# semicolonTransistor/rust-ray-tracing

Measured on AMD Instinct MI355X. Metric: Msamples/s (pixels×spp/s), 1920×1080·512spp·500 spheres; 1/2/4/8 GPU, higher is better.
Workload: dtype f32

## Files before the change

rust-ray-tracing_amd/csrc/rt_trace.hpp:

```cpp
#pragma once
#include "rt_sweep.hpp"
#include "rt_camera.hpp"
#include "rt_finish.hpp"

namespace rt {

struct IssueState { uint32_t busy, cur, cur_next, cur_pix, cur_row, cur_col, drained, qhead, qcount, blk_next, blk_end, need; };
struct IssueStateS { uint32_t busy, cur, cur_next, cur_pix, cur_row, cur_col, drained, qhead, qcount, blk_next, blk_end, need, cur_end; };

constexpr uint32_t kMaxBlock = 16;
constexpr uint32_t kBlockShare = 24;
constexpr uint32_t kClaimSpp = 640;
constexpr uint32_t kStreams = 8;
constexpr uint32_t kCtrStride = 64;

__device__ __forceinline__ bool guided_block(uint32_t np, uint32_t T, uint32_t G, uint32_t j, uint32_t& start,
                                             uint32_t& end) {
    uint32_t a = 0;
#pragma unroll
    for (uint32_t sz = kMaxBlock; sz >= 1u; sz >>= 1) {
        const uint32_t r = np - a, keep = sz * T;
        const uint32_t len = sz == 1u ? r : (sz <= G && r > keep ? ((r - keep) / sz) * sz : 0u);
        const uint32_t nb = len / sz;
        if (j < nb) { start = a + j * sz; end = start + sz; return true; }
        j -= nb;
        a += len;
    }
    return false;
}

constexpr uint32_t kQCap = 128;

template <typename T, bool B> constexpr bool kSplitKernel = B;

template <typename T, int W, bool ROOT2, int MODE = kModeV2, bool CAMQ = false, bool MEGA = false>
__global__ __launch_bounds__(256, W) void trace_paths(KParams<T> p) {
    constexpr bool SPLIT = kSplitKernel<T, false>, WIN = kSplitKernel<T, false>, ITEMS = kSplitKernel<T, false>;
    constexpr bool RAYS = kSplitKernel<T, false>;
#include "rt_trace_body.hpp"
}

template <typename T, int W, bool CAMQ, bool MEGA>
__global__ __launch_bounds__(256, W) void trace_paths_split(SParams<T> sp) {
    constexpr bool SPLIT = kSplitKernel<T, true>, WIN = kSplitKernel<T, false>, ITEMS = kSplitKernel<T, false>, ROOT2 = false;
    constexpr bool RAYS = kSplitKernel<T, false>;
    constexpr int MODE = kModeV2;
    const KParams<T>& p = sp.k;
#include "rt_trace_body.hpp"
}

template <typename T, int W, bool CAMQ, bool MEGA>
__global__ __launch_bounds__(256, W) void trace_paths_window(WParams<T> wp) {
    constexpr bool SPLIT = kSplitKernel<T, true>, WIN = kSplitKernel<T, true>, ITEMS = kSplitKernel<T, false>, ROOT2 = false;
    constexpr bool RAYS = kSplitKernel<T, false>;
    constexpr int MODE = kModeV2;
    const KParams<T>& p = wp.s.k;
#include "rt_trace_body.hpp"
}

template <typename T, int W, bool CAMQ, bool MEGA>
__global__ __launch_bounds__(256, W) void trace_paths_items(IParams<T> ip) {
    constexpr bool SPLIT = kSplitKernel<T, true>, WIN = kSplitKernel<T, false>, ITEMS = kSplitKernel<T, true>, ROOT2 = false;
    constexpr bool RAYS = kSplitKernel<T, false>;
    constexpr int MODE = kModeV2;
    const KParams<T>& p = ip.w.s.k;
#include "rt_trace_body.hpp"
}

template <typename T>
__global__ __launch_bounds__(256) void finish_records(SParams<T> sp) {
    __shared__ __attribute__((aligned(16))) uint32_t s_hist[4][64];
    __shared__ __attribute__((aligned(16))) T s_stage[4][3][64];
    __shared__ __attribute__((aligned(16))) uint16_t s_lmap[4][kLMapCap > 0u ? kLMapCap : 2];
    const uint32_t lane = threadIdx.x & 63u;
    const uint32_t wave = __builtin_amdgcn_readfirstlane(threadIdx.x >> 6);
    const auto& q = *cold_split_args<T>();
    const uint32_t gw = blockIdx.x * 4u + wave, nw = gridDim.x * 4u;
    const RScratch<T> sc{q.k.scratch + (size_t)gw * q.k.scratch_stride, q.rec, q.k.P, q.k.sbytes, q.k.swide};
    const uint32_t n_pix = q.n_pix;
    unsigned long long iters = 0;
    for (uint64_t px = gw; px < n_pix; px += nw) {
        iters += finish_pixel<T, kModeV2, true>(sc, (uint32_t)px, (uint32_t)px, s_hist[wave], s_stage[wave],
                                                kLMapCap > 0u ? s_lmap[wave] : nullptr, false);
        __builtin_amdgcn_wave_barrier();
    }
    if (lane == 0 && iters != 0ull) atomicAdd(&q.k.segs[(gw & (kSegShards - 1)) * kSegStride + 2], iters);
}

template <typename T>
__global__ __launch_bounds__(256) void finish_window(WParams<T> wp) {
    __shared__ __attribute__((aligned(16))) uint32_t s_hist[4][64];
    __shared__ __attribute__((aligned(16))) T s_stage[4][3][64];
    __shared__ __attribute__((aligned(16))) uint16_t s_lmap[4][kLMapCap > 0u ? kLMapCap : 2];
    const uint32_t lane = threadIdx.x & 63u;
    const uint32_t wave = __builtin_amdgcn_readfirstlane(threadIdx.x >> 6);
    const auto& q = *cold_split_args<T>();
    const uint32_t gw = blockIdx.x * 4u + wave, nw = gridDim.x * 4u;
    const RScratch<T> sc{q.k.scratch + (size_t)gw * q.k.scratch_stride, q.rec, cold_window_args<T>()->P_cap, q.k.sbytes,
                         q.k.swide};
    const uint32_t n_pix = q.n_pix;
    unsigned long long iters = 0;
    for (uint64_t px = gw; px < n_pix; px += nw) {
        iters += finish_pixel<T, kModeV2, true>(sc, (uint32_t)px, (uint32_t)px, s_hist[wave], s_stage[wave],
                                                kLMapCap > 0u ? s_lmap[wave] : nullptr, false);
        __builtin_amdgcn_wave_barrier();
    }
    if (lane == 0 && iters != 0ull) atomicAdd(&q.k.segs[(gw & (kSegShards - 1)) * kSegStride + 2], iters);
}

template <typename T>
__global__ __launch_bounds__(256) void finish_window_list(LParams<T> lp) {
    __shared__ __attribute__((aligned(16))) uint32_t s_hist[4][64];
    __shared__ __attribute__((aligned(16))) T s_stage[4][3][64];
    __shared__ __attribute__((aligned(16))) uint16_t s_lmap[4][kLMapCap > 0u ? kLMapCap : 2];
    const uint32_t lane = threadIdx.x & 63u;
    const uint32_t wave = __builtin_amdgcn_readfirstlane(threadIdx.x >> 6);
    const auto& q = *cold_split_args<T>();
    const uint32_t gw = blockIdx.x * 4u + wave, nw = gridDim.x * 4u;
    const RScratch<T> sc{q.k.scratch + (size_t)gw * q.k.scratch_stride, q.rec, cold_window_args<T>()->P_cap, q.k.sbytes,
                         q.k.swide};
    const uint32_t n_list = q.n_pix;
    const cptr<uint32_t> list = (cptr<uint32_t>)cold_list_args<T>()->list;
    unsigned long long iters = 0;
    for (uint64_t i = gw; i < n_list; i += nw) {
        const uint32_t px = list[i];
        iters += finish_pixel<T, kModeV2, true>(sc, px, px, s_hist[wave], s_stage[wave],
                                                kLMapCap > 0u ? s_lmap[wave] : nullptr, false);
        __builtin_amdgcn_wave_barrier();
    }
    if (lane == 0 && iters != 0ull) atomicAdd(&q.k.segs[(gw & (kSegShards - 1)) * kSegStride + 2], iters);
}

__global__ __launch_bounds__(256) void progressive_error(const double* full, const double* half,
                                                         const uint32_t* counts, double* out, uint32_t n) {
    const uint32_t i = blockIdx.x * 256u + threadIdx.x;
    if (i >= n) return;
    double e = __builtin_huge_val();
    if (counts[i] >= 2u) {
        e = 0.0;
        for (uint32_t ch = 0; ch < 3u; ++ch) e = fmax(e, fabs(full[3u * i + ch] - half[3u * i + ch]));
    }
    out[i] = e;
}

constexpr uint32_t kRefineBlock = 256;

__device__ inline uint32_t refine_block_scan(uint32_t v, uint32_t* buf, uint32_t* total) {
    const uint32_t t = threadIdx.x;
    buf[t] = v;
    __syncthreads();
    for (uint32_t d = 1; d < kRefineBlock; d <<= 1) {
        const uint32_t a = t >= d ? buf[t - d] : 0u;
        __syncthreads();
        buf[t] += a;
        __syncthreads();
    }
    const uint32_t incl = buf[t];
    *total = buf[kRefineBlock - 1];
    __syncthreads();
    return incl - v;
}

__global__ __launch_bounds__(256) void refine_select(const uint32_t* list, uint32_t n, uint32_t count, double tol,
                                                     uint32_t may_grow, double* cur, const double* fresh,
                                                     uint32_t* counts, uint8_t* flags, uint32_t* blk) {
    __shared__ uint32_t s_buf[kRefineBlock];
    const uint32_t i = blockIdx.x * kRefineBlock + threadIdx.x;
    uint32_t act = 0u;
    if (i < n) {
        const size_t p = list ? list[i] : i;
        double e = __builtin_huge_val();
        if (count >= 2u) {
            e = 0.0;
            for (uint32_t ch = 0; ch < 3u; ++ch) e = fmax(e, fabs(fresh[3u * p + ch] - cur[3u * p + ch]));
        }
        for (uint32_t ch = 0; ch < 3u; ++ch) cur[3u * p + ch] = fresh[3u * p + ch];
        act = (e > tol && may_grow != 0u) ? 1u : 0u;
        counts[p] = count;
        flags[i] = (uint8_t)act;
    }
    uint32_t total = 0u;
    (void)refine_block_scan(act, s_buf, &total);
    if (threadIdx.x == 0u) blk[blockIdx.x] = total;
}

__global__ __launch_bounds__(256) void refine_scan(uint32_t* blk, uint32_t nb, uint32_t* ret) {
    __shared__ uint32_t s_buf[kRefineBlock];
    uint32_t carry = 0u;
    for (uint32_t base = 0; base < nb; base += kRefineBlock) {
        const uint32_t idx = base + threadIdx.x;
        const uint32_t v = idx < nb ? blk[idx] : 0u;
        uint32_t total = 0u;
        const uint32_t ex = refine_block_scan(v, s_buf, &total);
        if (idx < nb) blk[idx] = carry + ex;
        carry += total;
    }
    if (threadIdx.x < 4u) ret[threadIdx.x] = threadIdx.x == 0u ? carry : 0u;
}

__global__ __launch_bounds__(256) void refine_scatter(const uint32_t* list, uint32_t n, const uint8_t* flags,
                                                      const uint32_t* off, uint32_t* next, uint32_t* retired) {
    __shared__ uint32_t s_buf[kRefineBlock];
    const uint32_t first = blockIdx.x * kRefineBlock, i = first + threadIdx.x;
    const uint32_t act = i < n ? (uint32_t)flags[i] : 0u;
    uint32_t total = 0u;
    const uint32_t rank = refine_block_scan(act, s_buf, &total);
    if (i >= n) return;
    const uint32_t p = list ? list[i] : i;
    const uint32_t a0 = off[blockIdx.x];
    if (act) next[a0 + rank] = p;
    else retired[(first - a0) + (threadIdx.x - rank)] = p;
}

__global__ __launch_bounds__(256) void refine_expand(const uint32_t* act, uint32_t n_act, uint32_t* counts,
                                                     uint32_t done, uint32_t target, uint32_t base, uint32_t S,
                                                     uint32_t nsub, MapItem* items) {
    const uint32_t i = blockIdx.x * kRefineBlock + threadIdx.x;
    if (i >= n_act) return;
    const uint32_t p = act[i];
    counts[p] = target;
    for (uint32_t j = 0; j < nsub; ++j) {
        const uint32_t a = base + j * S, b = a + S;
        items[(size_t)i * nsub + j] = MapItem{p, a > done ? a : done, b < target ? b : target, 0u};
    }
}

}
```

rust-ray-tracing_amd/csrc/rt_trace_body.hpp:

```cpp
    constexpr bool SC = MODE == kModeScalar;
    static_assert(!SPLIT || (MODE == kModeV2 && !ROOT2), "the sample-parallel kernels cover the live path only");
    static_assert(!ITEMS || (SPLIT && !WIN), "an item table replaces the window's decode");
    static_assert(!RAYS || (!SPLIT && !CAMQ && MODE == kModeV2), "caller rays: the live path, one item per pixel, no camera batches");
    constexpr bool kF64Park = sizeof(T) == 8 && W >= 5;
    constexpr uint32_t QW = CAMQ ? 4 : 1, QN = CAMQ ? (kF64Park ? 64u : kQCap) : 1;
    __shared__ unsigned long long wcount[4][4];
    __shared__ __attribute__((aligned(16))) uint32_t s_hist[4][64];
    __shared__ __attribute__((aligned(16))) T s_stage[4][3][64];
    using IS = std::conditional_t<SPLIT, IssueStateS, IssueState>;
    __shared__ IS s_is[4];
    __shared__ unsigned long long s_pool;
    __shared__ uint32_t s_dry;
    __shared__ uint32_t q_sid[QW][QN];
    __shared__ uint32_t s_slotpix[4][kSlots];
    __shared__ uint32_t s_item[4][kSlots];
    __shared__ int q_hit[QW][QN];
    __shared__ T q_t[QW][QN], q_d[QW][3][QN];
    __shared__ alignas(16) uint16_t s_clist[QW][CAMQ ? kSlots : 1][kCList];
    constexpr bool kPark = (sizeof(T) == 4 && W >= 6) || kF64Park;
    constexpr bool kParkC = kPark && (MEGA || (sizeof(T) == 4 && W == 6));
    __shared__ T s_park[kPark ? 4 : 1][kParkC ? 9 : 6][64];
    constexpr bool kLMap = MODE == kModeV2 && !MEGA && kLMapCap > 0u && sizeof(T) == 8 && !kF64Park;
    __shared__ __attribute__((aligned(16))) uint16_t s_lmap[kLMap ? 4 : 1][kLMap ? kLMapCap : 2];
    const uint32_t lane = threadIdx.x & 63u;
    const uint32_t wave = __builtin_amdgcn_readfirstlane(threadIdx.x >> 6);
    if (lane == 0) { wcount[wave][0] = 0; wcount[wave][1] = 0; wcount[wave][2] = 0; wcount[wave][3] = 0; }
    if (lane < kNWork) g_work[wave][lane] = 0ull;
#ifdef RT_KSTATS
    if (lane < kNKstat) g_kst[wave][lane] = 0;
#endif
    if constexpr (SPLIT) {
        if (lane == 0) s_is[wave] = IssueStateS{};
    } else {
        if (lane == 0) s_is[wave] = IssueState{0u, 0u, cold_args<T>()->spp, 0u, 0u, 0u, 0u, 0u, 0u, 0u, 0u, 0u};
    }
    {
        const auto& q = *cold_args<T>();
        uint32_t b0 = 0, b1 = 0;
        const bool got = guided_block(q.n_items, max(1u, kTMul * gridDim.x), q.blk_g, blockIdx.x, b0, b1);
        if (threadIdx.x == 0) {
            s_pool = got ? ((unsigned long long)b0 << 32) | b1 : 0ull;
            s_dry = 0u;
        }
    }
    __syncthreads();
    V3<T> o = mk(T(0), T(0), T(0)), d = o, c = o;
    uint32_t ss = 0, k = 0;
    constexpr bool kParkSS = MEGA;
    uint32_t* const ssp = (uint32_t*)&s_stage[wave][0][0] + lane;
    auto ss_get = [&]() -> uint32_t {
        if constexpr (kParkSS) { asm volatile("" ::: "memory"); return *ssp; }
        else return ss;
    };
    auto ss_set = [&](uint32_t v) {
        if constexpr (kParkSS) *ssp = v;
        else ss = v;
    };
    if constexpr (kParkSS) *ssp = 0u;
    constexpr uint32_t kSlotNZ = 0x80000000u;
    uint32_t slot_left = 0;
    auto sid_of = [](uint32_t v) -> uint32_t { return v & 0x1FFFFFFFu; };
    auto slot_of = [](uint32_t v) -> uint32_t { return v >> 29; };
    bool live = false;
    bool scat = false;
    int hit_i = -1;
    T hit_t = T(0);
    auto park = [&](const V3<T>& po, const V3<T>& pd) {
        T* r = &s_park[kPark ? wave : 0][0][lane];
        r[0] = po.x; r[64] = po.y; r[128] = po.z; r[192] = pd.x; r[256] = pd.y; r[320] = pd.z;
    };
    auto unpark = [&](V3<T>& po, V3<T>& pd) {
        asm volatile("" ::: "memory");
        const T* r = &s_park[kPark ? wave : 0][0][lane];
        po = mk(r[0], r[64], r[128]);
        pd = mk(r[192], r[256], r[320]);
    };
    auto park_c = [&](const V3<T>& pc) {
        T* r = &s_park[kPark ? wave : 0][kParkC ? 6 : 0][lane];
        r[0] = pc.x; r[64] = pc.y; r[128] = pc.z;
    };
    auto unpark_c = [&]() -> V3<T> {
        asm volatile("" ::: "memory");
        const T* r = &s_park[kPark ? wave : 0][kParkC ? 6 : 0][lane];
        return mk(r[0], r[64], r[128]);
    };

    constexpr bool kDirectSky = CAMQ && MODE == kModeV2 && !SPLIT;
    auto issue = [&](unsigned long long want, uint32_t& i_sid, uint32_t& i_slot, uint32_t& i_pix,
                     uint32_t& i_row, uint32_t& i_col) -> bool {
        const uint32_t spp = cold_args<T>()->spp;
        bool got = false;
        uint32_t busy = __builtin_amdgcn_readfirstlane(s_is[wave].busy);
        uint32_t cur = __builtin_amdgcn_readfirstlane(s_is[wave].cur);
        uint32_t cur_next = __builtin_amdgcn_readfirstlane(s_is[wave].cur_next);
        uint32_t cur_pix = __builtin_amdgcn_readfirstlane(s_is[wave].cur_pix);
        uint32_t cur_row = __builtin_amdgcn_readfirstlane(s_is[wave].cur_row);
        uint32_t cur_col = __builtin_amdgcn_readfirstlane(s_is[wave].cur_col);
        bool drained = __builtin_amdgcn_readfirstlane(s_is[wave].drained) != 0u;
        uint32_t blk_next = __builtin_amdgcn_readfirstlane(s_is[wave].blk_next);
        uint32_t blk_end = __builtin_amdgcn_readfirstlane(s_is[wave].blk_end);
        uint32_t opened = 0, listed = 0;
        uint32_t cur_end = spp;
        if constexpr (SPLIT) cur_end = __builtin_amdgcn_readfirstlane(s_is[wave].cur_end);
        while (want != 0ull && !drained) {
            if (cur_next == cur_end) {
                const uint32_t avail = ~busy & ((1u << kSlots) - 1u);
                if (avail == 0u) break;
                const auto& q = *cold_args<T>();
                uint32_t item = blk_next;
                if (blk_next < blk_end) {
                    ++blk_next;
                } else {
                    uint32_t it = 0xFFFFFFFFu, nb = 0, ne = 0;
                    if (lane == 0) {
                        unsigned long long pv = __hip_atomic_load(&s_pool, __ATOMIC_RELAXED, __HIP_MEMORY_SCOPE_WORKGROUP);
                        for (;;) {
                            if ((uint32_t)(pv >> 32) >= (uint32_t)pv) break;
                            const unsigned long long old = atomicCAS(&s_pool, pv, pv + (1ull << 32));
                            if (old == pv) { it = (uint32_t)(pv >> 32); break; }
                            pv = old;
                        }
                        uint32_t b0 = 0, b1 = 0;
                        bool claimed = false;
                        for (uint32_t r = 0; it == 0xFFFFFFFFu && r < kStreams && !claimed; ++r) {
                            const uint32_t s = (blockIdx.x + r) % kStreams;
                            if ((__hip_atomic_load(&s_dry, __ATOMIC_RELAXED, __HIP_MEMORY_SCOPE_WORKGROUP) >> s) & 1u) continue;
                            const uint32_t j = gridDim.x + s + kStreams * atomicAdd(q.counter + kCtrStride * s, 1u);
                            claimed = guided_block(q.n_items, max(1u, kTMul * gridDim.x), q.blk_g, j, b0, b1);
                            if (!claimed) atomicOr(&s_dry, 1u << s);
                        }
                        if (claimed) {
                            it = b0;
                            if (b1 > b0 + 1u && atomicCAS(&s_pool, pv, ((unsigned long long)(b0 + 1u) << 32) | b1) != pv) {
                                nb = b0 + 1u;
                                ne = b1;
                            }
                        }
                    }
                    it = __builtin_amdgcn_readfirstlane(it);
                    if (it == 0xFFFFFFFFu) { drained = true; break; }
                    item = it;
                    blk_next = __builtin_amdgcn_readfirstlane(nb);
                    blk_end = __builtin_amdgcn_readfirstlane(ne);
                }
                const uint32_t s = __builtin_ctz(avail);
                uint32_t first = 0;
                if constexpr (ITEMS) {
                    const cptr<MapItem> tab = (cptr<MapItem>)__builtin_assume_aligned(cold_items_args<T>()->items, 16);
                    first = tab[item].first;
                    cur_end = tab[item].end;
                    item = tab[item].pixel;
                } else if constexpr (SPLIT) {
                    const auto& sq = *cold_split_args<T>();
                    const uint32_t px = item / sq.nsub;
                    first = (item - px * sq.nsub) * sq.S;
                    if constexpr (WIN) {
                        const auto& wq = *cold_window_args<T>();
                        first += wq.s_base;
                        cur_end = min(spp, first + sq.S);
                        first = max(first, wq.s_begin);
                    } else {
                        cur_end = min(spp, first + sq.S);
                    }
                    item = px;
                }
                if constexpr (RAYS) {
                    const auto& rq = *cold_rays_args<T>();
                    cur_row = 0u;
                    cur_col = 0u;
                    cur_pix = rq.pixel_base + item;
                    const cptr<uint64_t> skip = (cptr<uint64_t>)__builtin_assume_aligned(rq.skip, 8);
                    if ((skip[item >> 6] >> (item & 63u)) & 1ull) continue;
                } else {
                    const uint32_t ri = item / q.col_count, ci = item % q.col_count;
                    cur_row = q.row_begin + ri * q.row_step;
                    cur_col = q.col_begin + ci;
                    cur_pix = cur_row * q.W + cur_col;
                }
                if constexpr (kDirectSky) {
                    if (cold_args<T>()->depth > 1u) {
                        const uint32_t nl = pixel_list<T, MEGA>(cur_col, cur_row, s_clist[wave][s]);
                        if (nl == 0u) {
                            const uint32_t ss_keep = kParkSS ? *ssp : 0u;
                            finish_sky_direct<T>(item, cur_col, cur_row, cur_pix, s_hist[wave], s_stage[wave]);
                            if constexpr (kParkSS) {
                                __builtin_amdgcn_wave_barrier();
                                *ssp = ss_keep;
                            }
                            if (lane == 0) { wcount[wave][0] += spp; wcount[wave][3] += spp; wcount[wave][2] += 1u; }
                            continue;
                        }
                        listed |= 1u << s;
                    }
                }
                if (lane == 0) { s_slotpix[wave][s] = cur_pix; s_item[wave][s] = item; }
                if (lane == s) slot_left = cur_end - first;
                busy |= 1u << s;
                opened |= 1u << s;
                cur = s;
                cur_next = first;
            }
            const bool isw = (want >> lane) & 1ull;
            const uint32_t take = min((uint32_t)__popcll(want), cur_end - cur_next);
            const uint32_t r = lanes_below(want);
            const bool mine = isw && r < take;
            if (mine) { got = true; i_sid = cur_next + r; i_slot = cur; i_pix = cur_pix; i_row = cur_row; i_col = cur_col; }
            want &= ~__ballot(mine);
            cur_next += take;
        }
        if (lane == 0) {
            s_is[wave].busy = busy; s_is[wave].cur = cur; s_is[wave].cur_next = cur_next; s_is[wave].cur_pix = cur_pix;
            s_is[wave].cur_row = cur_row; s_is[wave].cur_col = cur_col; s_is[wave].drained = drained ? 1u : 0u;
            s_is[wave].blk_next = blk_next; s_is[wave].blk_end = blk_end;
            if (CAMQ) s_is[wave].need |= opened & ~listed;
            if constexpr (SPLIT) s_is[wave].cur_end = cur_end;
        }
        return got;
    };

    auto terminate = [&](bool term, bool skyhit, uint32_t e, uint32_t t_slot, uint32_t t_sid, const V3<T>& tc,
                         const V3<T>& td) {
        if constexpr (SPLIT) {
            if (term) {
                const RScratch<T> sc = split_records<T>();
                const uint32_t px = s_item[wave][t_slot];
                sc.set_e(px, t_sid, e);
                if (skyhit && e != 0u) sc.store_c(px, t_sid, tc.x, tc.y, tc.z);
            }
        } else if (term) {
            const PScratch<T> sc = wave_scratch<T>(wave);
            sc.set_e(t_slot, t_sid, e);
            if (MODE == kModeV2) {
                if (skyhit && e != 0u) sc.store_c(t_slot, t_sid, tc.x, tc.y, tc.z);
            } else {
                V3<T> v = mk(T(0.0), T(0.0), T(0.0));
                if (skyhit) { const V3<T> sk = sky(td.y); v = mk(tc.x * sk.x, tc.y * sk.y, tc.z * sk.z); }
                sc.store_c(t_slot, t_sid, v.x, v.y, v.z);
            }
        }
        unsigned long long tm = __ballot(term);
        const unsigned long long nzl = MODE == kModeV2 && !SPLIT ? __ballot(term && e != 0u) : 0ull;
        bool synced = false;
        while (tm != 0ull) {
            const uint32_t s = __builtin_amdgcn_readlane(t_slot, __builtin_ctzll(tm));
            const unsigned long long m = __ballot(term && t_slot == s);
            tm &= ~m;
            if (lane == s) slot_left = (slot_left - (uint32_t)__popcll(m)) | ((m & nzl) != 0ull ? kSlotNZ : 0u);
            const uint32_t left = __builtin_amdgcn_readlane(slot_left, s);
            if constexpr (SPLIT) {
                if (left == 0u) {
                    const uint32_t b = __builtin_amdgcn_readfirstlane(s_is[wave].busy);
                    if (lane == 0) s_is[wave].busy = b & ~(1u << s);
                }
            } else if (__builtin_expect((left & ~kSlotNZ) == 0u, 0)) {
                const uint32_t ss_keep = kParkSS ? *ssp : 0u;
                if (!synced) { wave_mem_sync(); synced = true; }
                KSTAT(6);
                const uint32_t K = finish_pixel<T, MODE, !MEGA>(
                    wave_scratch<T>(wave), s, __builtin_amdgcn_readfirstlane(s_item[wave][s]), s_hist[wave], s_stage[wave],
                    kLMap ? s_lmap[wave] : nullptr, (left & kSlotNZ) == 0u);
                if constexpr (kParkSS) {
                    __builtin_amdgcn_wave_barrier();
                    *ssp = ss_keep;
                }
                if (lane == 0) wcount[wave][2] += K;
                const uint32_t b = __builtin_amdgcn_readfirstlane(s_is[wave].busy);
                if (lane == 0) s_is[wave].busy = b & ~(1u << s);
            }
        }
    };

    auto camera_batch = [&]() -> bool {
        uint32_t bsid = 0, bslot = 0, bpix = 0, brow = 0, bcol = 0;
        const bool v = issue(~0ull, bsid, bslot, bpix, brow, bcol);
        const unsigned long long vm = __ballot(v);
        if (vm == 0ull) return false;
        V3<T> bd = mk(T(0), T(0), T(0));
        if (v) {
            const U4 r = [&] {
                const auto& q0 = *cold_args<T>();
                return rng<T>(bsid, bpix, 0u, 0u, q0.k0, q0.k1);
            }();
            const auto& q = *cold_args_after<T>(r.a ^ r.b);
            const T s1 = div_dim((T)bcol + u01a(r, T(0)), q.W, q.rW);
            const T s2 = div_dim((T)brow + u01b(r, T(0)), q.H, q.rH);
            const V3<T> vu = mk(q.vu[0], q.vu[1], q.vu[2]), vv = mk(q.vv[0], q.vv[1], q.vv[2]);
            const V3<T> pc = add(mk(q.ulc[0], q.ulc[1], q.ulc[2]), add(mul(vu, s1), mul(vv, s2)));
            bd = unit(sub(pc, mk(q.center[0], q.center[1], q.center[2])));
            if constexpr (SPLIT) split_records<T>().y(s_item[wave][bslot], bsid) = bd.y;
            else if (MODE == kModeV2) wave_scratch<T>(wave).y(bslot, bsid) = bd.y;
        }
        T bt = T(0);
        int bi = -1;
        {
            uint32_t smask = 0;
            for (unsigned long long m = vm; m != 0ull;) {
                const uint32_t sl = __builtin_amdgcn_readlane(bslot, (int)__builtin_ctzll(m));
                smask |= 1u << sl;
                m &= ~__ballot(v && bslot == sl);
            }
            uint32_t need = __builtin_amdgcn_readfirstlane(s_is[wave].need) & smask;
            if (need != 0u) {
                if (lane == 0) s_is[wave].need = s_is[wave].need & ~need;
                const uint32_t iw = cold_args<T>()->W;
                while (need != 0u) {
                    const uint32_t sl = (uint32_t)__builtin_ctz(need);
                    need &= need - 1u;
                    const uint32_t pxi = __builtin_amdgcn_readfirstlane(s_slotpix[wave][sl]);
                    const uint32_t row = pxi / iw;
                    (void)pixel_list<T, MEGA>(pxi - row * iw, row, s_clist[wave][sl]);
                }
            }
            bool listed = true;
            for (uint32_t m = smask; m != 0u; m &= m - 1u)
                if (__builtin_amdgcn_readfirstlane(s_clist[wave][__builtin_ctz(m)][0]) == 0xFFFFu) listed = false;
            if (listed) bi = camera_listed<T, ROOT2, SC>(v, bd, bt, s_clist[wave], smask);
            else bi = camera_sweep<T, ROOT2, SC, MEGA>(v, bd, bt);
        }
        if (lane == 0) { wcount[wave][0] += (uint32_t)__popcll(vm); wcount[wave][1] += 64u; }
        const uint32_t depth = cold_args<T>()->depth;
        const bool skyhit = v && bi < 0;
        const bool term = v && (skyhit || depth == 1u);
        const bool push = v && !term;
        const unsigned long long pm = __ballot(push);
        const uint32_t qhead = __builtin_amdgcn_readfirstlane(s_is[wave].qhead);
        const uint32_t qcount = __builtin_amdgcn_readfirstlane(s_is[wave].qcount);
        if (push) {
            const uint32_t e = (qhead + qcount + lanes_below(pm)) % QN;
            q_sid[wave][e] = bsid | (bslot << 29);
            q_hit[wave][e] = bi;
            q_t[wave][e] = bt;
            q_d[wave][0][e] = bd.x; q_d[wave][1][e] = bd.y; q_d[wave][2][e] = bd.z;
        }
        if (lane == 0) s_is[wave].qcount = qcount + (uint32_t)__popcll(pm);
        terminate(term, skyhit, skyhit ? 0u : depth, bslot, bsid, mk(T(1.0), T(1.0), T(1.0)), bd);
        return true;
    };

    for (;;) {
        bool fresh = false;
        uint32_t frow = 0, fcol = 0, npix = 0;
        if constexpr (CAMQ) {
            const unsigned long long freem = __ballot(!live);
            const uint32_t nfree = (uint32_t)__popcll(freem);
            for (;;) {
                const uint32_t qcount = __builtin_amdgcn_readfirstlane(s_is[wave].qcount);
                if (qcount >= nfree || qcount + 64u > QN) break;
                if (!camera_batch()) break;
            }
            const uint32_t qhead = __builtin_amdgcn_readfirstlane(s_is[wave].qhead);
            const uint32_t qcount = __builtin_amdgcn_readfirstlane(s_is[wave].qcount);
            const uint32_t take = min(nfree, qcount);
            const uint32_t r = lanes_below(freem);
            if (!live && r < take) {
                const uint32_t e = (qhead + r) % QN;
                ss_set(q_sid[wave][e]);
                hit_i = q_hit[wave][e];
                hit_t = q_t[wave][e];
                const auto& q = *cold_args<T>();
                const V3<T> pd = mk(q_d[wave][0][e], q_d[wave][1][e], q_d[wave][2][e]);
                const V3<T> po = mk(q.center[0], q.center[1], q.center[2]);
                if constexpr (kPark) park(po, pd);
                else { d = pd; o = po; }
                if constexpr (kParkC) park_c(mk(T(1.0), T(1.0), T(1.0)));
                else c = mk(T(1.0), T(1.0), T(1.0));
                k = 0;
                live = true;
                scat = true;
            }
            if (lane == 0) { s_is[wave].qhead = (qhead + take) % QN; s_is[wave].qcount = qcount - take; }
        } else {
            uint32_t nsid = 0, nslot = 0;
            fresh = issue(__ballot(!live), nsid, nslot, npix, frow, fcol);
            if (fresh) ss_set(nsid | (nslot << 29));
        }
        if constexpr (kPark) unpark(o, d);
        if constexpr (kParkC) c = unpark_c();
        if (fresh || scat) {
            const uint32_t ssv = ss_get();
            const uint32_t pix = (!CAMQ && fresh) ? npix : s_slotpix[wave][slot_of(ssv)];
            if constexpr (RAYS) {
                if (fresh) {
                    const auto& rq = *cold_rays_args<T>();
                    const size_t ray = (size_t)(pix - rq.pixel_base) * rq.R + sid_of(ssv) % rq.R;
                    const T* dp = rq.directions + 3 * ray;
                    d = mk(dp[0], dp[1], dp[2]);
                    if (rq.origins != nullptr) {
                        const T* op = rq.origins + 3 * ray;
                        o = mk(op[0], op[1], op[2]);
                    } else {
                        o = mk(rq.k.center[0], rq.k.center[1], rq.k.center[2]);
                    }
                    c = mk(T(1.0), T(1.0), T(1.0));
                } else {
                    next_ray<T, SC>(false, fcol, frow, pix, sid_of(ssv), k, hit_i, hit_t, o, d, c);
                }
            } else {
                next_ray<T, SC>(CAMQ ? false : fresh, fcol, frow, pix, sid_of(ssv), k, hit_i, hit_t, o, d, c);
            }
        }
        if constexpr (kPark) park(o, d);
        if constexpr (kParkC) park_c(c);
        if (fresh) {
            k = 0;
            live = true;
            if constexpr (SPLIT) {
                const uint32_t ssv = ss_get();
                split_records<T>().y(s_item[wave][slot_of(ssv)], sid_of(ssv)) = d.y;
            } else if (MODE == kModeV2) {
                const uint32_t ssv = ss_get();
                wave_scratch<T>(wave).y(slot_of(ssv), sid_of(ssv)) = d.y;
            }
        } else if (scat) {
            k += 1u;
        }
        if (__ballot(live) == 0ull) break;
        const uint32_t depth = cold_args<T>()->depth;
        const bool act = live && k < depth;
        hit_i = -1;
        if (act) hit_i = nearest_hit<T, ROOT2, SC, false, MEGA>(p, o, d, hit_t);
        const unsigned long long bact = __ballot(act);
        if (lane == 0 && bact) { wcount[wave][0] += (uint32_t)__popcll(bact); wcount[wave][1] += 64u; }
        const bool skyhit = act && hit_i < 0;
        const bool term = live && (!act || skyhit || k + 1 == depth);
        scat = act && hit_i >= 0 && k + 1 < depth;
        if constexpr (kPark) {
            if (MODE != kModeV2) { V3<T> po, pd; unpark(po, pd); d = pd; }
        }
        if constexpr (kParkC) c = unpark_c();
        {
            const uint32_t ssv = ss_get();
            terminate(term, skyhit, skyhit ? k : depth, slot_of(ssv), sid_of(ssv), c, d);
        }
        live = live && !term;
    }
    if (lane == 0) {
        const auto& q = *cold_args<T>();
        const uint32_t gw = blockIdx.x * (blockDim.x >> 6) + wave;
        unsigned long long* cc = &q.segs[(gw & (kSegShards - 1)) * kSegStride];
        atomicAdd(cc + 0, wcount[wave][0]);
        atomicAdd(cc + 1, wcount[wave][1]);
        atomicAdd(cc + 2, wcount[wave][2]);
        if (wcount[wave][3]) atomicAdd(cc + kDirectSkySlot, wcount[wave][3]);
        for (uint32_t i = 0; i < kNWork; ++i) atomicAdd(cc + kWorkSlot + i, g_work[wave][i]);
#ifdef RT_KSTATS
        for (int i = 0; i < kNKstat; ++i) atomicAdd(cc + kstat_slot(i), g_kst[wave][i]);
#endif
    }
```

Measured before the change: 40030.

## Pack per-wave issue state into bitfields and add a fast issue path

Compacts the per-wave issue state in LDS into packed flags (busy, need, no-list, current slot, drained) and a combined queue head/count word. It also adds an early-exit fast path when the current pixel has enough samples left for every requesting lane. The issue function now returns the mask of slots it used, which replaces the per-batch ballot loop and the scan of clist headers. The aim is fewer LDS reads and writes and less scalar bookkeeping per issue and per camera batch, at the cost of more intricate bit manipulation and a tighter limit on slot count.

```diff
diff --git a/rust-ray-tracing_amd/csrc/rt_trace.hpp b/rust-ray-tracing_amd/csrc/rt_trace.hpp
--- a/rust-ray-tracing_amd/csrc/rt_trace.hpp
+++ b/rust-ray-tracing_amd/csrc/rt_trace.hpp
@@ -5,8 +5,11 @@
 
 namespace rt {
 
-struct IssueState { uint32_t busy, cur, cur_next, cur_pix, cur_row, cur_col, drained, qhead, qcount, blk_next, blk_end, need; };
-struct IssueStateS { uint32_t busy, cur, cur_next, cur_pix, cur_row, cur_col, drained, qhead, qcount, blk_next, blk_end, need, cur_end; };
+struct alignas(16) IssueState { uint32_t cur_next, cur_pix, cur_row, cur_col, flags, q, blk_next, blk_end; };
+struct alignas(16) IssueStateS { uint32_t cur_next, cur_pix, cur_row, cur_col, flags, q, blk_next, blk_end, cur_end; };
+constexpr uint32_t kISBusy = 0, kISNeed = 8, kISNoList = 16, kISCur = 24;
+constexpr uint32_t kISDrained = 1u << 27;
+static_assert(kSlots <= 8u, "a slot mask is 8 bits of IssueState::flags, a slot index 3");
 
 constexpr uint32_t kMaxBlock = 16;
 constexpr uint32_t kBlockShare = 24;
diff --git a/rust-ray-tracing_amd/csrc/rt_trace_body.hpp b/rust-ray-tracing_amd/csrc/rt_trace_body.hpp
--- a/rust-ray-tracing_amd/csrc/rt_trace_body.hpp
+++ b/rust-ray-tracing_amd/csrc/rt_trace_body.hpp
@@ -32,7 +32,7 @@
     if constexpr (SPLIT) {
         if (lane == 0) s_is[wave] = IssueStateS{};
     } else {
-        if (lane == 0) s_is[wave] = IssueState{0u, 0u, cold_args<T>()->spp, 0u, 0u, 0u, 0u, 0u, 0u, 0u, 0u, 0u};
+        if (lane == 0) s_is[wave] = IssueState{cold_args<T>()->spp, 0u, 0u, 0u, 0u, 0u, 0u, 0u};
     }
     {
         const auto& q = *cold_args<T>();
@@ -87,24 +87,32 @@
 
     constexpr bool kDirectSky = CAMQ && MODE == kModeV2 && !SPLIT;
     auto issue = [&](unsigned long long want, uint32_t& i_sid, uint32_t& i_slot, uint32_t& i_pix,
-                     uint32_t& i_row, uint32_t& i_col) -> bool {
+                     uint32_t& i_row, uint32_t& i_col, uint32_t& i_mask) -> bool {
+        i_mask = 0u;
+        if (want == 0ull) return false;
         const uint32_t spp = cold_args<T>()->spp;
-        bool got = false;
-        uint32_t busy = __builtin_amdgcn_readfirstlane(s_is[wave].busy);
-        uint32_t cur = __builtin_amdgcn_readfirstlane(s_is[wave].cur);
         uint32_t cur_next = __builtin_amdgcn_readfirstlane(s_is[wave].cur_next);
+        uint32_t cur_end = spp;
+        if constexpr (SPLIT) cur_end = __builtin_amdgcn_readfirstlane(s_is[wave].cur_end);
+        uint32_t flags = __builtin_amdgcn_readfirstlane(s_is[wave].flags);
         uint32_t cur_pix = __builtin_amdgcn_readfirstlane(s_is[wave].cur_pix);
         uint32_t cur_row = __builtin_amdgcn_readfirstlane(s_is[wave].cur_row);
         uint32_t cur_col = __builtin_amdgcn_readfirstlane(s_is[wave].cur_col);
-        bool drained = __builtin_amdgcn_readfirstlane(s_is[wave].drained) != 0u;
+        uint32_t cur = (flags >> kISCur) & 7u;
+        const uint32_t nwant = (uint32_t)__popcll(want);
+        if (cur_end - cur_next >= nwant) {
+            const bool isw = (want >> lane) & 1ull;
+            if (isw) { i_sid = cur_next + lanes_below(want); i_slot = cur; i_pix = cur_pix; i_row = cur_row; i_col = cur_col; }
+            if (lane == 0) s_is[wave].cur_next = cur_next + nwant;
+            i_mask = 1u << cur;
+            return isw;
+        }
+        bool got = false;
         uint32_t blk_next = __builtin_amdgcn_readfirstlane(s_is[wave].blk_next);
         uint32_t blk_end = __builtin_amdgcn_readfirstlane(s_is[wave].blk_end);
-        uint32_t opened = 0, listed = 0;
-        uint32_t cur_end = spp;
-        if constexpr (SPLIT) cur_end = __builtin_amdgcn_readfirstlane(s_is[wave].cur_end);
-        while (want != 0ull && !drained) {
+        while (want != 0ull && (flags & kISDrained) == 0u) {
             if (cur_next == cur_end) {
-                const uint32_t avail = ~busy & ((1u << kSlots) - 1u);
+                const uint32_t avail = ~(flags >> kISBusy) & ((1u << kSlots) - 1u);
                 if (avail == 0u) break;
                 const auto& q = *cold_args<T>();
                 uint32_t item = blk_next;
@@ -138,12 +146,13 @@
                         }
                     }
                     it = __builtin_amdgcn_readfirstlane(it);
-                    if (it == 0xFFFFFFFFu) { drained = true; break; }
+                    if (it == 0xFFFFFFFFu) { flags |= kISDrained; break; }
                     item = it;
                     blk_next = __builtin_amdgcn_readfirstlane(nb);
                     blk_end = __builtin_amdgcn_readfirstlane(ne);
                 }
                 const uint32_t s = __builtin_ctz(avail);
+                uint32_t sbits = (1u << (kISBusy + s)) | (CAMQ ? 1u << (kISNeed + s) : 0u);
                 uint32_t first = 0;
                 if constexpr (ITEMS) {
                     const cptr<MapItem> tab = (cptr<MapItem>)__builtin_assume_aligned(cold_items_args<T>()->items, 16);
@@ -179,7 +188,7 @@
                 }
                 if constexpr (kDirectSky) {
                     if (cold_args<T>()->depth > 1u) {
-                        const uint32_t nl = pixel_list<T, MEGA>(cur_col, cur_row, s_clist[wave][s]);
+                        const uint32_t nl = __builtin_amdgcn_readfirstlane(pixel_list<T, MEGA>(cur_col, cur_row, s_clist[wave][s]));
                         if (nl == 0u) {
                             const uint32_t ss_keep = kParkSS ? *ssp : 0u;
                             finish_sky_direct<T>(item, cur_col, cur_row, cur_pix, s_hist[wave], s_stage[wave]);
@@ -190,13 +199,12 @@
                             if (lane == 0) { wcount[wave][0] += spp; wcount[wave][3] += spp; wcount[wave][2] += 1u; }
                             continue;
                         }
-                        listed |= 1u << s;
+                        sbits = (1u << (kISBusy + s)) | ((nl == 0xFFFFu ? 1u : 0u) << (kISNoList + s));
                     }
                 }
                 if (lane == 0) { s_slotpix[wave][s] = cur_pix; s_item[wave][s] = item; }
                 if (lane == s) slot_left = cur_end - first;
-                busy |= 1u << s;
-                opened |= 1u << s;
+                flags = (flags & ~((1u << (kISNeed + s)) | (1u << (kISNoList + s)) | (7u << kISCur))) | sbits | (s << kISCur);
                 cur = s;
                 cur_next = first;
             }
@@ -207,12 +215,12 @@
             if (mine) { got = true; i_sid = cur_next + r; i_slot = cur; i_pix = cur_pix; i_row = cur_row; i_col = cur_col; }
             want &= ~__ballot(mine);
             cur_next += take;
+            i_mask |= (take != 0u ? 1u : 0u) << cur;
         }
         if (lane == 0) {
-            s_is[wave].busy = busy; s_is[wave].cur = cur; s_is[wave].cur_next = cur_next; s_is[wave].cur_pix = cur_pix;
-            s_is[wave].cur_row = cur_row; s_is[wave].cur_col = cur_col; s_is[wave].drained = drained ? 1u : 0u;
-            s_is[wave].blk_next = blk_next; s_is[wave].blk_end = blk_end;
-            if (CAMQ) s_is[wave].need |= opened & ~listed;
+            s_is[wave].cur_next = cur_next; s_is[wave].cur_pix = cur_pix; s_is[wave].cur_row = cur_row;
+            s_is[wave].cur_col = cur_col; s_is[wave].flags = flags; s_is[wave].blk_next = blk_next;
+            s_is[wave].blk_end = blk_end;
             if constexpr (SPLIT) s_is[wave].cur_end = cur_end;
         }
         return got;
@@ -249,8 +257,8 @@
             const uint32_t left = __builtin_amdgcn_readlane(slot_left, s);
             if constexpr (SPLIT) {
                 if (left == 0u) {
-                    const uint32_t b = __builtin_amdgcn_readfirstlane(s_is[wave].busy);
-                    if (lane == 0) s_is[wave].busy = b & ~(1u << s);
+                    const uint32_t b = __builtin_amdgcn_readfirstlane(s_is[wave].flags);
+                    if (lane == 0) s_is[wave].flags = b & ~(1u << (kISBusy + s));
                 }
             } else if (__builtin_expect((left & ~kSlotNZ) == 0u, 0)) {
                 const uint32_t ss_keep = kParkSS ? *ssp : 0u;
@@ -264,15 +272,16 @@
                     *ssp = ss_keep;
                 }
                 if (lane == 0) wcount[wave][2] += K;
-                const uint32_t b = __builtin_amdgcn_readfirstlane(s_is[wave].busy);
-                if (lane == 0) s_is[wave].busy = b & ~(1u << s);
+                const uint32_t b = __builtin_amdgcn_readfirstlane(s_is[wave].flags);
+                if (lane == 0) s_is[wave].flags = b & ~(1u << (kISBusy + s));
             }
         }
     };
 
     auto camera_batch = [&]() -> bool {
         uint32_t bsid = 0, bslot = 0, bpix = 0, brow = 0, bcol = 0;
-        const bool v = issue(~0ull, bsid, bslot, bpix, brow, bcol);
+        uint32_t smask = 0;
+        const bool v = issue(~0ull, bsid, bslot, bpix, brow, bcol, smask);
         const unsigned long long vm = __ballot(v);
         if (vm == 0ull) return false;
         V3<T> bd = mk(T(0), T(0), T(0));
@@ -293,27 +302,22 @@
         T bt = T(0);
         int bi = -1;
         {
-            uint32_t smask = 0;
-            for (unsigned long long m = vm; m != 0ull;) {
-                const uint32_t sl = __builtin_amdgcn_readlane(bslot, (int)__builtin_ctzll(m));
-                smask |= 1u << sl;
-                m &= ~__ballot(v && bslot == sl);
-            }
-            uint32_t need = __builtin_amdgcn_readfirstlane(s_is[wave].need) & smask;
+            uint32_t fl = __builtin_amdgcn_readfirstlane(s_is[wave].flags);
+            uint32_t need = (fl >> kISNeed) & smask;
             if (need != 0u) {
-                if (lane == 0) s_is[wave].need = s_is[wave].need & ~need;
+                fl &= ~(need << kISNeed);
                 const uint32_t iw = cold_args<T>()->W;
                 while (need != 0u) {
                     const uint32_t sl = (uint32_t)__builtin_ctz(need);
                     need &= need - 1u;
                     const uint32_t pxi = __builtin_amdgcn_readfirstlane(s_slotpix[wave][sl]);
                     const uint32_t row = pxi / iw;
-                    (void)pixel_list<T, MEGA>(pxi - row * iw, row, s_clist[wave][sl]);
-                }
-            }
-            bool listed = true;
-            for (uint32_t m = smask; m != 0u; m &= m - 1u)
-                if (__builtin_amdgcn_readfirstlane(s_clist[wave][__builtin_ctz(m)][0]) == 0xFFFFu) listed = false;
+                    const uint32_t nl = __builtin_amdgcn_readfirstlane(pixel_list<T, MEGA>(pxi - row * iw, row, s_clist[wave][sl]));
+                    if (nl == 0xFFFFu) fl |= 1u << (kISNoList + sl);
+                }
+                if (lane == 0) s_is[wave].flags = fl;
+            }
+            const bool listed = ((fl >> kISNoList) & smask) == 0u;
             if (listed) bi = camera_listed<T, ROOT2, SC>(v, bd, bt, s_clist[wave], smask);
             else bi = camera_sweep<T, ROOT2, SC, MEGA>(v, bd, bt);
         }
@@ -323,8 +327,8 @@
         const bool term = v && (skyhit || depth == 1u);
         const bool push = v && !term;
         const unsigned long long pm = __ballot(push);
-        const uint32_t qhead = __builtin_amdgcn_readfirstlane(s_is[wave].qhead);
-        const uint32_t qcount = __builtin_amdgcn_readfirstlane(s_is[wave].qcount);
+        const uint32_t q = __builtin_amdgcn_readfirstlane(s_is[wave].q);
+        const uint32_t qhead = q & 0xFFFFu, qcount = q >> 16;
         if (push) {
             const uint32_t e = (qhead + qcount + lanes_below(pm)) % QN;
             q_sid[wave][e] = bsid | (bslot << 29);
@@ -332,7 +336,7 @@
             q_t[wave][e] = bt;
             q_d[wave][0][e] = bd.x; q_d[wave][1][e] = bd.y; q_d[wave][2][e] = bd.z;
         }
-        if (lane == 0) s_is[wave].qcount = qcount + (uint32_t)__popcll(pm);
+        if (lane == 0) s_is[wave].q = q + ((uint32_t)__popcll(pm) << 16);
         terminate(term, skyhit, skyhit ? 0u : depth, bslot, bsid, mk(T(1.0), T(1.0), T(1.0)), bd);
         return true;
     };
@@ -343,13 +347,16 @@
         if constexpr (CAMQ) {
             const unsigned long long freem = __ballot(!live);
             const uint32_t nfree = (uint32_t)__popcll(freem);
+            uint32_t q = 0;
             for (;;) {
-                const uint32_t qcount = __builtin_amdgcn_readfirstlane(s_is[wave].qcount);
-                if (qcount >= nfree || qcount + 64u > QN) break;
-                if (!camera_batch()) break;
-            }
-            const uint32_t qhead = __builtin_amdgcn_readfirstlane(s_is[wave].qhead);
-            const uint32_t qcount = __builtin_amdgcn_readfirstlane(s_is[wave].qcount);
+                q = __builtin_amdgcn_readfirstlane(s_is[wave].q);
+                if ((q >> 16) >= nfree || (q >> 16) + 64u > QN) break;
+                if (!camera_batch()) {
+                    q = __builtin_amdgcn_readfirstlane(s_is[wave].q);
+                    break;
+                }
+            }
+            const uint32_t qhead = q & 0xFFFFu, qcount = q >> 16;
             const uint32_t take = min(nfree, qcount);
             const uint32_t r = lanes_below(freem);
             if (!live && r < take) {
@@ -368,10 +375,10 @@
                 live = true;
                 scat = true;
             }
-            if (lane == 0) { s_is[wave].qhead = (qhead + take) % QN; s_is[wave].qcount = qcount - take; }
+            if (lane == 0) s_is[wave].q = ((qhead + take) % QN) | ((qcount - take) << 16);
         } else {
-            uint32_t nsid = 0, nslot = 0;
-            fresh = issue(__ballot(!live), nsid, nslot, npix, frow, fcol);
+            uint32_t nsid = 0, nslot = 0, nmask = 0;
+            fresh = issue(__ballot(!live), nsid, nslot, npix, frow, fcol, nmask);
             if (fresh) ss_set(nsid | (nslot << 29));
         }
         if constexpr (kPark) unpark(o, d);
```

Result: faster. 41460 (median of 6 runs) (+3.6%).
